# drtconway/zotmer

Hardware: AMD Instinct MI355X
Metric: Gk-mers/sec kmerize k=25 on synthetic 150bp FASTQ; achieved HBM GB/s fraction (higher is better)
Workload: dtype u64

## Files before the change

zotmer_amd/csrc/dedupe2.hip:

```cpp
#include "dedupe.hpp"
#include <type_traits>

namespace zk {

template <int BLOCK_, int BATCH_, int ITEMS_>
struct Dedupe2Smem {
    static constexpr int BLOCK = BLOCK_, BATCH = BATCH_, ITEMS = ITEMS_, TILE = BLOCK * ITEMS, NW = BLOCK / 64, ALL = 11264, SPT = ALL / BLOCK,
                         NB = 1024, SIDE = 64 + 64 * BATCH;
    static_assert(ALL % BLOCK == 0 && ALL % 8 == 0 && ITEMS % BATCH == 0 && ITEMS % 4 == 0, "whole rounds, whole quads, whole batches");
    alignas(16) u32 keys[ALL];
    alignas(16) u32 cnt[ALL / 2];
    union {
        u32 side[NW][SIDE];
        struct { u32 bc[NB]; u32 bbase[NB + 1]; } g;
    };
    u32 ticket;
    u32 nout;
};
template <int BLOCK_, int BATCH_, int ITEMS_>
struct Dedupe2MirrorSmem : Dedupe2Smem<BLOCK_, BATCH_, ITEMS_> {
    u32 bins[2][MIRROR_RADIX];
    u64 mbase;
};

template <int ITEMS>
struct Dedupe2Next {
    u32 chunk;
    u64 lo;
    u32 len;
    u32 tag[ITEMS];
};

template <int BLOCK, int ITEMS, bool TAGIN>
__device__ __forceinline__ void dedupe2_load(const DedupeArgs& a, u64 lo, u32 pos, u32 rem, u32 tmask, u32 (&t)[ITEMS]) {
    constexpr u32 TILE = BLOCK * ITEMS;
    u32 tid = threadIdx.x;
    asm volatile("" : "+v"(tid));
    if constexpr (TAGIN) {
        const u32* tp = a.tin + lo + pos;
        if (rem >= TILE) {
            struct __attribute__((packed, aligned(4))) Tag4 { u32 a, b, c, d; };
            static_assert(ITEMS % 4 == 0, "whole quads");
#pragma unroll
            for (int i = 0; i < ITEMS / 4; i++) {
                const Tag4 q = *reinterpret_cast<const Tag4*>(tp + (u32)i * (4 * BLOCK) + 4 * tid);
                t[4 * i] = q.a; t[4 * i + 1] = q.b; t[4 * i + 2] = q.c; t[4 * i + 3] = q.d;
            }
        } else {
#pragma unroll
            for (int i = 0; i < ITEMS; i++) {
                const u32 g = (u32)i * BLOCK + tid;
                t[i] = g < rem ? tp[g] : 0u;
            }
        }
    } else {
        const u64* kp = a.kin + lo + pos;
#pragma unroll
        for (int i = 0; i < ITEMS; i++) {
            const u32 g = (u32)i * BLOCK + tid;
            t[i] = g < rem ? (u32)kp[g] & tmask : 0u;
        }
    }
}

template <class S, bool TAGIN, bool UNSORTED, bool MIRROR>
__device__ __forceinline__ void dedupe2_block(const DedupeArgs& a, S& sm, Dedupe2Next<S::ITEMS>& st, u32 (&ph)[8], u32& tlast) {
    constexpr int BLOCK = S::BLOCK, BATCH = S::BATCH, ITEMS = S::ITEMS, TILE = S::TILE, ALL = S::ALL, SPT = S::SPT, NB = S::NB;
    static_assert(!MIRROR || UNSORTED, "the mirror words are written beside the unsorted ones");
    constexpr u32 EMPTY = ~0u;
    constexpr u32 HS = ALL - 1;
    int tid = threadIdx.x;
    asm volatile("" : "+v"(tid));
    const int lane = tid & 63, wave = __builtin_amdgcn_readfirstlane(tid >> 6);
    const u32 chunk = st.chunk;
    const u64 lo = st.lo;
    const u32 len = st.len;
    const u32 maxc = (1u << a.pack) - 1u;
    const u32 tmask = a.tag_bits >= 32 ? ~0u : (1u << a.tag_bits) - 1u;
    auto next_block = [&](u32 t) {
        st.chunk = t; st.lo = 0; st.len = 0;
        if (t < a.chunks) {
            const u64 nlo = a.cuts[t], nhi = a.cuts[t + 1];
            st.lo = nlo;
            st.len = nhi - nlo < (u64)a.limit ? (u32)(nhi - nlo) : ~0u;
        }
        if (st.len - 1u < ~0u - 1u) dedupe2_load<BLOCK, ITEMS, TAGIN>(a, st.lo, 0, st.len, tmask, st.tag);
    };
    if (tid == 0) sm.ticket = atomicAdd(a.counter, 1u);
    if (len == 0 || len == ~0u) {
        if (tid == 0) {
            if (len) a.retry[atomicAdd(a.n_retry, 1u)] = chunk;
            a.nwords[chunk] = 0;
        }
        if (a.sub && tid < 64) a.sub[(u64)chunk * 64 + tid] = 0;
        __syncthreads();
        next_block((u32)__builtin_amdgcn_readfirstlane((int)sm.ticket));
        return;
    }
    for (int q = tid; q < ALL / 4; q += BLOCK) reinterpret_cast<uint4*>(sm.keys)[q] = make_uint4(~0u, ~0u, ~0u, ~0u);
    for (int q = tid; q < ALL / 8; q += BLOCK) reinterpret_cast<uint4*>(sm.cnt)[q] = make_uint4(0, 0, 0, 0);
    if (UNSORTED && tid == 0) sm.nout = 0;
    __syncthreads();
    DD_PHASE(0);
    const u32 nchunk = (u32)__builtin_amdgcn_readfirstlane((int)sm.ticket);
    u32 bad = 0;
    u32 nside = 0;
    auto home = [&](u32 e) -> u32 {
        u32 hh = __umulhi(e * 0x9E3779B1u, HS);
        asm("" : "+v"(hh));
        return e == EMPTY ? HS : hh;
    };
    auto count = [&](u32 h, u32 inc) { atomicAdd(&sm.cnt[h >> 1], inc << ((h & 1u) << 4)); };
    auto drain = [&](u32 from, u32 n) {
        if ((u32)lane < n) {
            const u32 e = sm.side[wave][from + lane];
            u32 h = home(e) + 1;
            h = h >= HS ? 0u : h;
            int p = 0;
            for (; p < ALL; p++) {
                const u32 old = atomicCAS(&sm.keys[h], EMPTY, e);
                if (old == EMPTY || old == e) break;
                h = h + 1 == HS ? 0u : h + 1;
            }
            if (p < ALL) count(h, 1u); else bad = 1;
        }
    };
    auto insert = [&](auto whole, const u32 (&e)[BATCH], const bool (&valid)[BATCH]) {
        constexpr bool WHOLE = decltype(whole)::value;
        u32 h[BATCH], old[BATCH];
#pragma unroll
        for (int j = 0; j < BATCH; j++) h[j] = home(e[j]);
#pragma unroll
        for (int j = 0; j < BATCH; j++) old[j] = (WHOLE || valid[j]) ? atomicCAS(&sm.keys[h[j]], EMPTY, e[j]) : e[j];
#pragma unroll
        for (int j = 0; j < BATCH; j++) {
            const bool ok = old[j] == EMPTY || old[j] == e[j];
            count(h[j], (ok && (WHOLE || valid[j])) ? 1u : 0u);
            const u64 m = __ballot(!ok);
            if (!ok) sm.side[wave][nside + popc_below(m)] = e[j];
            nside += (u32)__popcll(m);
        }
        while (nside >= 64) { nside -= 64; drain(nside, 64); }
    };
    u32 tag[ITEMS], nt[ITEMS];
#pragma unroll
    for (int i = 0; i < ITEMS; i++) tag[i] = st.tag[i];
    for (u32 pos = 0; pos < len; pos += TILE) {
        const u32 rem = len - pos;
        if (rem > (u32)TILE) dedupe2_load<BLOCK, ITEMS, TAGIN>(a, lo, pos + TILE, rem - TILE, tmask, nt);
#pragma unroll
        for (int i0 = 0; i0 < ITEMS; i0 += BATCH) {
            u32 e[BATCH];
            bool valid[BATCH];
#pragma unroll
            for (int j = 0; j < BATCH; j++) { e[j] = tag[i0 + j]; valid[j] = (u32)(i0 + j) * BLOCK + tid < rem; }
            if (rem >= (u32)TILE) insert(std::true_type(), e, valid); else insert(std::false_type(), e, valid);
        }
#pragma unroll
        for (int i = 0; i < ITEMS; i++) tag[i] = nt[i];
    }
    drain(0, nside);
    DD_PHASE(1);
    const int any_bad = __syncthreads_or((int)bad);
    DD_PHASE(2);
    if (any_bad) {
        if (tid == 0) {
            a.retry[atomicAdd(a.n_retry, 1u)] = chunk;
            a.nwords[chunk] = 0;
        }
        if (a.sub && tid < 64) a.sub[(u64)chunk * 64 + tid] = 0;
        next_block(nchunk);
        return;
    }
    if constexpr (UNSORTED) {
        if constexpr (!MIRROR) next_block(nchunk);
        const u16* cnt16 = reinterpret_cast<const u16*>(sm.cnt);
        u32 wn = 0;
#pragma unroll
        for (int j = 0; j < SPT; j++) wn += (u32)__popcll(__ballot(cnt16[tid + j * BLOCK] != 0));
        u32 wbase = 0;
        if (lane == 0 && wn) wbase = atomicAdd(&sm.nout, wn);
        wbase = (u32)__shfl((int)wbase, 0, 64);
        u32 mrun = 0;
        u64* mp = nullptr;
        u64* op = nullptr;
        if constexpr (MIRROR) {
            __syncthreads();
            u64 g = 0;
            if (tid == 0) g = atomicAdd(a.m_cursor, (u64)sm.nout);
            next_block(nchunk);
            if (tid == 0) sm.mbase = g;
            __syncthreads();
            const u64 mb = sm.mbase;
            const u64 mbase = ((u64)(u32)__builtin_amdgcn_readfirstlane((int)(mb >> 32)) << 32) | (u64)(u32)__builtin_amdgcn_readfirstlane((int)mb);
            const u32 wb = (u32)__builtin_amdgcn_readfirstlane((int)wbase);
            op = a.out + lo + wb;
            if (mbase + sm.nout <= a.m_cap) mp = a.m_out + mbase + wb;
            else if (tid == 0) atomicOr(a.flags, 4u);
        }
        DD_PHASE(3);
        const u64 hi_part = (u64)chunk << a.tag_bits;
#pragma unroll
        for (int j = 0; j < SPT; j++) {
            const u32 c = cnt16[tid + j * BLOCK];
            const u64 bal = __ballot(c != 0);
            if (c) {
                const u64 k = hi_part | (u64)sm.keys[tid + j * BLOCK];
                if (c > maxc) {
                    const u32 at = atomicAdd(a.n_big, 1u);
                    if (at < a.big_cap) { a.big[2 * (u64)at] = k; a.big[2 * (u64)at + 1] = c; }
                    atomicOr(a.flags, 2u);
                }
                const u64 cw = (u64)(c > maxc ? 0u : c);
                if constexpr (MIRROR) op[mrun + popc_below(bal)] = (k << a.pack) | cw;
                else a.out[lo + wbase + popc_below(bal)] = (k << a.pack) | cw;
                if constexpr (MIRROR) {
                    if (mp) {
                        const u64 mw = (revcomp(a.m_K, k) << a.pack) | cw;
                        mp[mrun + popc_below(bal)] = mw;
                        const u32 top = (u32)(mw >> a.m_shift[0]);
                        atomicAdd(&sm.bins[0][top & ((1u << a.m_bits[0]) - 1u)], 1u);
                        atomicAdd(&sm.bins[1][(top >> a.m_bits[0]) & (MIRROR_RADIX - 1)], 1u);
                    }
                }
            }
            if constexpr (MIRROR) mrun += (u32)__popcll(bal);
            else wbase += (u32)__popcll(bal);
        }
        __syncthreads();
        if (tid == 0) a.nwords[chunk] = sm.nout;
        DD_PHASE(5);
        return;
    }
    for (int q = tid; q < NB; q += BLOCK) sm.g.bc[q] = 0;
    u32 et[SPT], ec[SPT];
    const int gb = a.tag_bits < 10 ? a.tag_bits : 10, bsh = a.tag_bits - gb;
    const u16* cnt16 = reinterpret_cast<const u16*>(sm.cnt);
#pragma unroll
    for (int j = 0; j < SPT; j++) {
        et[j] = sm.keys[tid + j * BLOCK];
        ec[j] = cnt16[tid + j * BLOCK];
    }
    __syncthreads();
#pragma unroll
    for (int j = 0; j < SPT; j++) {
        if (ec[j]) ec[j] |= atomicAdd(&sm.g.bc[(et[j] >> bsh) & (NB - 1)], 1u) << 16;
        if (j % 6 == 5) __builtin_amdgcn_sched_barrier(0);
    }
    __syncthreads();
    DD_PHASE(3);
    if (wave == 0) {
        constexpr int PER = NB / 64;
        u32 cs[PER], sum = 0;
#pragma unroll
        for (int r = 0; r < PER; r++) { cs[r] = sm.g.bc[PER * lane + r]; sum += cs[r]; }
        const u32 inc = wave_incl_scan_u32(sum);
        u32 run = inc - sum;
#pragma unroll
        for (int r = 0; r < PER; r++) { sm.g.bbase[PER * lane + r] = run; run += cs[r]; }
        if (lane == 63) sm.g.bbase[NB] = inc;
    }
    __syncthreads();
    const u32 total = sm.g.bbase[NB];
    if (tid == 0) a.nwords[chunk] = total;
    if (a.sub && tid < 64) a.sub[(u64)chunk * 64 + tid] = sm.g.bbase[16 * tid + 16] - sm.g.bbase[16 * tid];
    u16* cw16 = reinterpret_cast<u16*>(sm.cnt);
#pragma unroll
    for (int j = 0; j < SPT; j++) {
        if (ec[j]) {
            const u32 p = sm.g.bbase[(et[j] >> bsh) & (NB - 1)] + (ec[j] >> 16);
            sm.keys[p] = et[j];
            cw16[p] = (u16)ec[j];
        }
    }
    __syncthreads();
    DD_PHASE(4);
    next_block(nchunk);
    const u64 hi_part = (u64)chunk << a.tag_bits;
    constexpr int E = 3;
    for (u32 i0 = (u32)tid; i0 < total; i0 += E * BLOCK) {
        u32 mine[E], cc[E], g0[E], g1[E], rank[E];
#pragma unroll
        for (int e = 0; e < E; e++) {
            const u32 i = i0 + e * BLOCK;
            mine[e] = sm.keys[i < total ? i : 0u];
            cc[e] = cnt16[i < total ? i : 0u];
        }
#pragma unroll
        for (int e = 0; e < E; e++) {
            const u32 b = (mine[e] >> bsh) & (NB - 1);
            g0[e] = sm.g.bbase[b]; g1[e] = sm.g.bbase[b + 1];
        }
        u32 o[E][4];
#pragma unroll
        for (int e = 0; e < E; e++)
#pragma unroll
            for (int r = 0; r < 4; r++) o[e][r] = sm.keys[g0[e] + r < (u32)ALL ? g0[e] + r : (u32)ALL - 1];
#pragma unroll
        for (int e = 0; e < E; e++) {
            rank[e] = 0;
#pragma unroll
            for (int r = 0; r < 4; r++) rank[e] += (g0[e] + r < g1[e] && o[e][r] < mine[e]) ? 1u : 0u;
            for (u32 q = g0[e] + 4; q < g1[e]; q += 4) {
                u32 p4[4];
#pragma unroll
                for (int r = 0; r < 4; r++) p4[r] = sm.keys[q + r < (u32)ALL ? q + r : (u32)ALL - 1];
#pragma unroll
                for (int r = 0; r < 4; r++) rank[e] += (q + r < g1[e] && p4[r] < mine[e]) ? 1u : 0u;
            }
        }
#pragma unroll
        for (int e = 0; e < E; e++) {
            const u32 i = i0 + e * BLOCK;
            if (i >= total) break;
            const u32 c = cc[e];
            const u64 k = hi_part | (u64)mine[e];
            if (c > maxc) {
                const u32 at = atomicAdd(a.n_big, 1u);
                if (at < a.big_cap) { a.big[2 * (u64)at] = k; a.big[2 * (u64)at + 1] = c; }
                atomicOr(a.flags, 2u);
            }
            a.out[lo + g0[e] + rank[e]] = (k << a.pack) | (u64)(c > maxc ? 0u : c);
        }
    }
    DD_PHASE(5);
}

template <int BLOCK, int BATCH, int ITEMS, bool TAGIN, bool UNSORTED, bool MIRROR = false>
__global__ __launch_bounds__(BLOCK, 2 * BLOCK / 256) void dedupe2_kernel(DedupeArgs a) {
    using S = typename std::conditional<MIRROR, Dedupe2MirrorSmem<BLOCK, BATCH, ITEMS>, Dedupe2Smem<BLOCK, BATCH, ITEMS>>::type;
    __shared__ S sm;
    static_assert(sizeof(S) <= 80 * 1024, "two workgroups per CU");
    Dedupe2Next<ITEMS> st;
    if constexpr (MIRROR)
        for (int q = threadIdx.x; q < 2 * MIRROR_RADIX; q += BLOCK) (&sm.bins[0][0])[q] = 0;
    if (threadIdx.x == 0) sm.ticket = atomicAdd(a.counter, 1u);
    __syncthreads();
    st.chunk = (u32)__builtin_amdgcn_readfirstlane((int)sm.ticket);
    st.lo = 0; st.len = 0;
    const u32 tmask = a.tag_bits >= 32 ? ~0u : (1u << a.tag_bits) - 1u;
    if (st.chunk < a.chunks) {
        const u64 nlo = a.cuts[st.chunk], nhi = a.cuts[st.chunk + 1];
        st.lo = nlo;
        st.len = nhi - nlo < (u64)a.limit ? (u32)(nhi - nlo) : ~0u;
    }
    if (st.len - 1u < ~0u - 1u) dedupe2_load<BLOCK, ITEMS, TAGIN>(a, st.lo, 0, st.len, tmask, st.tag);
    __syncthreads();
    u32 ph[8] = {0, 0, 0, 0, 0, 0, 0, 0};
    u32 tlast = a.dbg ? (u32)__builtin_amdgcn_s_memtime() : 0u;
    (void)tlast;
    u32 nblk = 0;
    while (st.chunk < a.chunks) {
        dedupe2_block<S, TAGIN, UNSORTED, MIRROR>(a, sm, st, ph, tlast);
        __syncthreads();
        DD_PHASE(6);
        nblk++;
    }
    if constexpr (MIRROR) {
        for (int q = threadIdx.x; q < a.m_passes * MIRROR_RADIX; q += BLOCK) {
            const u32 x = (&sm.bins[0][0])[q];
            if (x) atomicAdd(&a.m_hist[q], (u64)x);
        }
    }
    if (a.dbg && threadIdx.x == 0 && blockIdx.x < 256) {
        for (int k = 0; k < 8; k++) a.dbg[(u64)blockIdx.x * 16 + k] = ph[k];
        a.dbg[(u64)blockIdx.x * 16 + 8] = nblk;
    }
}

int launch_dedupe2(zk_ctx* c, const DedupeArgs& a, bool tagin, int variant, bool unsorted) {
    const u32 want = 2u * (u32)c->num_cus;
    const u32 grid = a.chunks < want ? a.chunks : want;
    if (a.m_out) {
        if (!tagin || !unsorted || !a.m_cursor || !a.m_hist || a.m_passes < 1 || a.m_passes > 2 || a.m_bits[0] > MIRROR_RBITS || a.m_bits[1] > MIRROR_RBITS)
            return fail(c, ZK_EINTERNAL, "launch_dedupe2: mirror words with %d passes, tags %d, unsorted %d", a.m_passes, (int)tagin, (int)unsorted);
        if ((variant & 3) == 1) hipLaunchKernelGGL((dedupe2_kernel<512, 1, 8, true, true, true>), dim3(grid), dim3(512), 0, c->stream, a);
        else hipLaunchKernelGGL((dedupe2_kernel<512, 2, 8, true, true, true>), dim3(grid), dim3(512), 0, c->stream, a);
        ZK_HIP(c, hipGetLastError());
        return ZK_OK;
    }
#define ZK_DD2(N, T, U) hipLaunchKernelGGL((dedupe2_kernel<512, N, 8, T, U>), dim3(grid), dim3(512), 0, c->stream, a)
#define ZK_DD2B(T, U) switch (variant & 3) { case 1: ZK_DD2(1, T, U); break; case 2: ZK_DD2(2, T, U); break; default: ZK_DD2(4, T, U); break; }
    if (unsorted) {
        if (tagin) ZK_DD2B(true, true) else ZK_DD2B(false, true)
    } else {
        if (tagin) ZK_DD2B(true, false) else ZK_DD2B(false, false)
    }
#undef ZK_DD2B
#undef ZK_DD2
    ZK_HIP(c, hipGetLastError());
    return ZK_OK;
}

}
```

Measured before the change: 181.6.

## Compact nonzero counts per wave in LDS before emitting dense output

The unsorted output path now has each wave compact its own region of nonzero key/count slots in shared memory first, using ballot prefix sums. It then walks only the surviving entries in dense 64-lane batches to write output words. Before, every thread scanned all slots and lanes with zero counts sat idle during the global writes and mirror atomics. The cost is an extra LDS read/write pass, plus wave-private regions that need the static layout assumptions to hold.

```diff
diff --git a/zotmer_amd/csrc/dedupe2.hip b/zotmer_amd/csrc/dedupe2.hip
--- a/zotmer_amd/csrc/dedupe2.hip
+++ b/zotmer_amd/csrc/dedupe2.hip
@@ -174,14 +174,33 @@
     }
     if constexpr (UNSORTED) {
         if constexpr (!MIRROR) next_block(nchunk);
-        const u16* cnt16 = reinterpret_cast<const u16*>(sm.cnt);
+        constexpr int REG = ALL / S::NW, RPW = REG / 64;
+        constexpr int EC = 2, EW = 2;
+        static_assert(ALL % (S::NW * 64) == 0 && RPW % EC == 0 && REG % 2 == 0, "whole rounds a wave; no count word shared by two waves");
+        u16* cnt16 = reinterpret_cast<u16*>(sm.cnt);
+        const u32 base = (u32)(tid >> 6) * REG;
         u32 wn = 0;
 #pragma unroll
-        for (int j = 0; j < SPT; j++) wn += (u32)__popcll(__ballot(cnt16[tid + j * BLOCK] != 0));
+        for (int j0 = 0; j0 < RPW; j0 += EC) {
+            u32 ct[EC], cc[EC];
+#pragma unroll
+            for (int e = 0; e < EC; e++) {
+                ct[e] = sm.keys[base + (u32)(j0 + e) * 64 + lane];
+                cc[e] = cnt16[base + (u32)(j0 + e) * 64 + lane];
+            }
+#pragma unroll
+            for (int e = 0; e < EC; e++) asm volatile("" : "+v"(ct[e]), "+v"(cc[e]));
+#pragma unroll
+            for (int e = 0; e < EC; e++) {
+                const u64 bal = __ballot(cc[e] != 0);
+                const u32 dst = base + wn + popc_below(bal);
+                if (cc[e]) { sm.keys[dst] = ct[e]; cnt16[dst] = (u16)cc[e]; }
+                wn += (u32)__popcll(bal);
+            }
+        }
         u32 wbase = 0;
         if (lane == 0 && wn) wbase = atomicAdd(&sm.nout, wn);
         wbase = (u32)__shfl((int)wbase, 0, 64);
-        u32 mrun = 0;
         u64* mp = nullptr;
         u64* op = nullptr;
         if constexpr (MIRROR) {
@@ -193,39 +212,47 @@
             __syncthreads();
             const u64 mb = sm.mbase;
             const u64 mbase = ((u64)(u32)__builtin_amdgcn_readfirstlane((int)(mb >> 32)) << 32) | (u64)(u32)__builtin_amdgcn_readfirstlane((int)mb);
-            const u32 wb = (u32)__builtin_amdgcn_readfirstlane((int)wbase);
-            op = a.out + lo + wb;
-            if (mbase + sm.nout <= a.m_cap) mp = a.m_out + mbase + wb;
+            op = a.out + lo + wbase;
+            if (mbase + sm.nout <= a.m_cap) mp = a.m_out + mbase + wbase;
             else if (tid == 0) atomicOr(a.flags, 4u);
         }
+        else op = a.out + lo + wbase;
         DD_PHASE(3);
         const u64 hi_part = (u64)chunk << a.tag_bits;
-#pragma unroll
-        for (int j = 0; j < SPT; j++) {
-            const u32 c = cnt16[tid + j * BLOCK];
-            const u64 bal = __ballot(c != 0);
-            if (c) {
-                const u64 k = hi_part | (u64)sm.keys[tid + j * BLOCK];
-                if (c > maxc) {
-                    const u32 at = atomicAdd(a.n_big, 1u);
-                    if (at < a.big_cap) { a.big[2 * (u64)at] = k; a.big[2 * (u64)at + 1] = c; }
-                    atomicOr(a.flags, 2u);
-                }
-                const u64 cw = (u64)(c > maxc ? 0u : c);
-                if constexpr (MIRROR) op[mrun + popc_below(bal)] = (k << a.pack) | cw;
-                else a.out[lo + wbase + popc_below(bal)] = (k << a.pack) | cw;
-                if constexpr (MIRROR) {
-                    if (mp) {
-                        const u64 mw = (revcomp(a.m_K, k) << a.pack) | cw;
-                        mp[mrun + popc_below(bal)] = mw;
-                        const u32 top = (u32)(mw >> a.m_shift[0]);
-                        atomicAdd(&sm.bins[0][top & ((1u << a.m_bits[0]) - 1u)], 1u);
-                        atomicAdd(&sm.bins[1][(top >> a.m_bits[0]) & (MIRROR_RADIX - 1)], 1u);
+        for (u32 i0 = 0; i0 < wn; i0 += 64 * EW) {
+            u32 et[EW], ec[EW];
+#pragma unroll
+            for (int e = 0; e < EW; e++) {
+                const u32 i = i0 + (u32)e * 64 + lane;
+                et[e] = sm.keys[base + (i < wn ? i : 0u)];
+                ec[e] = cnt16[base + (i < wn ? i : 0u)];
+            }
+#pragma unroll
+            for (int e = 0; e < EW; e++) asm volatile("" : "+v"(et[e]), "+v"(ec[e]));
+#pragma unroll
+            for (int e = 0; e < EW; e++) {
+                const u32 i = i0 + (u32)e * 64 + lane;
+                if (i < wn) {
+                    const u32 c = ec[e];
+                    const u64 k = hi_part | (u64)et[e];
+                    if (c > maxc) {
+                        const u32 at = atomicAdd(a.n_big, 1u);
+                        if (at < a.big_cap) { a.big[2 * (u64)at] = k; a.big[2 * (u64)at + 1] = c; }
+                        atomicOr(a.flags, 2u);
+                    }
+                    const u64 cw = (u64)(c > maxc ? 0u : c);
+                    op[i] = (k << a.pack) | cw;
+                    if constexpr (MIRROR) {
+                        if (mp) {
+                            const u64 mw = (revcomp(a.m_K, k) << a.pack) | cw;
+                            mp[i] = mw;
+                            const u32 top = (u32)(mw >> a.m_shift[0]);
+                            atomicAdd(&sm.bins[0][top & ((1u << a.m_bits[0]) - 1u)], 1u);
+                            atomicAdd(&sm.bins[1][(top >> a.m_bits[0]) & (MIRROR_RADIX - 1)], 1u);
+                        }
                     }
                 }
             }
-            if constexpr (MIRROR) mrun += (u32)__popcll(bal);
-            else wbase += (u32)__popcll(bal);
         }
         __syncthreads();
         if (tid == 0) a.nwords[chunk] = sm.nout;
@@ -362,7 +389,9 @@
             if (x) atomicAdd(&a.m_hist[q], (u64)x);
         }
     }
-    if (a.dbg && threadIdx.x == 0 && blockIdx.x < 256) {
+    u32 tend = threadIdx.x;
+    asm volatile("" : "+v"(tend));
+    if (a.dbg && tend == 0 && blockIdx.x < 256) {
         for (int k = 0; k < 8; k++) a.dbg[(u64)blockIdx.x * 16 + k] = ph[k];
         a.dbg[(u64)blockIdx.x * 16 + 8] = nblk;
     }
```

Result: no change. 181.1 (-0.3%).
